# chanzuckerberg/shasta

Measured on NVIDIA H100. Metric: candidate_pairs_found_and_aligned_per_s, higher is better.
Workload: dtype u64/i32

## Files before the change

shasta_b200/csrc/align.cu:

```cuda
#include "context.cuh"
#include "align_kernels.cuh"
#include "hostpool.cuh"
#include "digest.cuh"

#include <algorithm>
#include <atomic>
#include <exception>
#include <memory>
#include <mutex>
#include <chrono>
#include <cstring>
#include <sys/mman.h>
#include <thread>
#include <limits>
#include <map>
#include <vector>

namespace shb {

extern thread_local uint64_t g_launchCount;

namespace {

uint32_t warpsForClass(const DpClass& k)
{
    if(k.c > 0) return kDpMaxWarpsPerBlock;
    const uint64_t perWarp = 3ull * (k.wMax + 1) * 4;
    const uint32_t w = uint32_t(std::min<uint64_t>(kDpMaxWarpsPerBlock, (200ull * 1024) / perWarp));
    return w ? w : 1;
}
size_t smemForClass(const DpClass& k, uint32_t warps) { return k.c > 0 ? 0 : size_t(warps) * 3 * (k.wMax + 1) * 4; }
size_t scanKernelSmemLimit()
{
    size_t most = 0;
    for(uint32_t k = 0; k < kDpClassCount; k++) most = std::max(most, smemForClass(dpClassAt(k), warpsForClass(dpClassAt(k))));
    return most;
}
constexpr uint32_t kMaxBandWidth = dpClassAt(kDpClassCount - 1).wMax;
struct DpLaunch { uint32_t blocks, threads; size_t smem; };
DpLaunch dpLaunch(const DpClass& k, uint32_t jobs)
{
    const uint32_t warps = warpsForClass(k);
    return DpLaunch{ceilDiv(jobs, warps * (32 / k.lanes)), warps * 32, smemForClass(k, warps)};
}

template<uint32_t K = 0, class... Args> void launchBanded(uint32_t k, const DpLaunch& l, cudaStream_t st, Args... args)
{
    if constexpr(K < kDpClassCount) {
        if(k != K) { launchBanded<K + 1>(k, l, st, args...); return; }
        constexpr DpClass cl = dpClassAt(K);
        if constexpr(cl.c == 0) {
            SHB_CUDA(cudaFuncSetAttribute(bandedAlignKernel<32, 0>, cudaFuncAttributeMaxDynamicSharedMemorySize, int(scanKernelSmemLimit())));
        }
        auto* kernel = &bandedAlignKernel<int(cl.lanes), int(cl.c)>;
        SHB_LAUNCH(kernel, l.blocks, l.threads, l.smem, st, args...);
    }
}
template<uint32_t K = 0, class... Args> void launchStage1Forward(uint32_t k, uint32_t jobs, cudaStream_t st, Args... args)
{
    if constexpr(K < kDpForwardClassCount) {
        if(k != K) { launchStage1Forward<K + 1>(k, jobs, st, args...); return; }
        constexpr DpForwardClass f = dpForwardClassAt(K);
        auto* kernel = &method3Stage1ForwardKernel<int(f.lanes), int(f.rows)>;
        SHB_LAUNCH(kernel, ceilDiv(jobs, kDpMaxWarpsPerBlock * (32 / f.lanes)), kDpMaxWarpsPerBlock * 32, 0, st, args...);
    }
}

struct Batch {
    DeviceBuffer<uint32_t> cand, counts, infoWords, jobKeep, jobBytes, keep, keepIndex, bytes32, selected;
    DeviceBuffer<DpJob> jobs1, jobs;
    DeviceBuffer<unsigned long long> tw, twOff, outCnt, outOff, bytes64, bytesOff, scanWs64;
    DeviceBuffer<uint32_t> trace;
    DeviceBuffer<uint2> ordinals, runs;
    DeviceBuffer<int2> endCells;
    DeviceBuffer<uint32_t> runCounts;
    DeviceBuffer<unsigned long long> cellCnt, cellOff;
    DeviceBuffer<uint32_t> gridCounts, gridAux, gridList, componentCount, jobOffsets;
    DeviceBuffer<uint8_t> gridFlags;
    DeviceBuffer<int32_t> gridBands;
    DeviceBuffer<uint32_t> orderValsA, orderValsB;
    DeviceBuffer<uint64_t> orderKeysA, orderKeysB;
    const uint32_t* order = nullptr;
};

enum WorkerScalar { kScTotal64 = 0, kScTotal32 = 1, kScSkipped = 2, kScForwardCells = 3, kScTooWide = 4, kScBandCells = 5,
                    kScDigits = 16, kScCount = 16 + 256 };

struct AlignWorker {
    cudaStream_t stream = nullptr;
    static constexpr int kSideStreams = 3;
    cudaStream_t side[kSideStreams] = {nullptr, nullptr, nullptr};
    cudaEvent_t forkEv = nullptr, joinEv[kSideStreams] = {nullptr, nullptr, nullptr};
    static constexpr int kHiStreams = 4;
    cudaStream_t hiStream[kHiStreams] = {nullptr, nullptr, nullptr, nullptr};
    cudaEvent_t hiJoinEv[kHiStreams] = {nullptr, nullptr, nullptr, nullptr};
    std::vector<cudaEvent_t> unitEvents;
    cudaEvent_t dp1a = nullptr, dp1b = nullptr, dp2a = nullptr, dp2b = nullptr;
    Batch batch;
    SortWorkspace sortWs;
    DeviceBuffer<uint32_t> scanWs;
    DeviceBuffer<unsigned long long> scalars;
    double dpMs = 0.;
    uint64_t traceWords = 0, launches = 0;

    void init()
    {
        if(stream) return;
        int least = 0, greatest = 0;
        SHB_CUDA(cudaDeviceGetStreamPriorityRange(&least, &greatest));
        SHB_CUDA(cudaStreamCreateWithFlags(&stream, cudaStreamNonBlocking));
        SHB_CUDA(cudaEventCreateWithFlags(&forkEv, cudaEventDisableTiming));
        for(int i = 0; i < kSideStreams; i++) {
            SHB_CUDA(cudaStreamCreateWithFlags(&side[i], cudaStreamNonBlocking));
            SHB_CUDA(cudaEventCreateWithFlags(&joinEv[i], cudaEventDisableTiming));
        }
        for(int i = 0; i < kHiStreams; i++) {
            SHB_CUDA(cudaStreamCreateWithPriority(&hiStream[i], cudaStreamNonBlocking, greatest));
            SHB_CUDA(cudaEventCreateWithFlags(&hiJoinEv[i], cudaEventDisableTiming));
        }
        SHB_CUDA(cudaEventCreate(&dp1a)); SHB_CUDA(cudaEventCreate(&dp1b));
        SHB_CUDA(cudaEventCreate(&dp2a)); SHB_CUDA(cudaEventCreate(&dp2b));
        scalars.reserve(kScCount);
    }
    ~AlignWorker()
    {
        for(int i = 0; i < kHiStreams; i++) { if(hiStream[i]) cudaStreamDestroy(hiStream[i]); if(hiJoinEv[i]) cudaEventDestroy(hiJoinEv[i]); }
        for(cudaEvent_t e : unitEvents) cudaEventDestroy(e);
        for(int i = 0; i < kSideStreams; i++) { if(side[i]) cudaStreamDestroy(side[i]); if(joinEv[i]) cudaEventDestroy(joinEv[i]); }
        for(cudaEvent_t e : {forkEv, dp1a, dp1b, dp2a, dp2b}) if(e) cudaEventDestroy(e);
        if(stream) cudaStreamDestroy(stream);
    }
    unsigned long long* sc(int k) { return scalars.get() + k; }
};

struct AlignCache {
    DeviceBuffer<uint64_t> dsToc;
    DeviceBuffer<uint32_t> dsKmer, dsOrdinal;
    uint32_t dsMaxRow = 0, dsK = 0;
    double dsFactor = -1.;
    uint64_t dsGeneration = ~0ull;
    DeviceBuffer<uint32_t> sortedKmer, sortedOrdinal;
    uint64_t sortedGeneration = ~0ull;
    uint64_t lengthCheckGeneration = ~0ull;
    uint64_t longestRead = 0;
    std::vector<std::unique_ptr<AlignWorker>> workers;
    DeviceBuffer<uint32_t> outRecords;
    DeviceBuffer<unsigned long long> outToc;
    DeviceBuffer<uint8_t> outData;
    cudaStream_t finalStream = nullptr;
    double lastBytesPerCandidate = 0.;
    ~AlignCache() { if(finalStream) cudaStreamDestroy(finalStream); }
};

AlignCache& cache(shb_context* c)
{
    if(!c->alignCache) c->alignCache = new AlignCache();
    return *static_cast<AlignCache*>(c->alignCache);
}

template<class F> void forEachClassConcurrently(AlignWorker& w, const std::vector<uint64_t>& classCounts, uint32_t chunkMax, F launch)
{
    cudaStream_t st = w.stream;
    struct Unit { int k; uint32_t count; uint64_t offset; };
    std::vector<Unit> units;
    const int classCount = int(classCounts.size());
    std::vector<uint64_t> offsets(classCounts.size(), 0);
    for(int k = 1; k < classCount; k++) offsets[k] = offsets[k-1] + classCounts[k-1];
    for(int k = classCount - 1; k >= 0; k--) {
        const uint64_t count = classCounts[k];
        if(!count) continue;
        const uint64_t chunks = (count + chunkMax - 1) / chunkMax, per = (count + chunks - 1) / chunks;
        for(uint64_t begin = 0; begin < count; begin += per) units.push_back({k, uint32_t(std::min(per, count - begin)), offsets[k] + begin});
    }
    if(units.empty()) return;
    constexpr int kStreams = AlignWorker::kSideStreams + 1;
    bool used[AlignWorker::kSideStreams] = {false, false, false};
    if(units.size() > 1) SHB_CUDA(cudaEventRecord(w.forkEv, st));
    for(size_t u = 0; u < units.size(); u++) {
        const int i = (u + 1 == units.size()) ? kStreams - 1 : int(u % kStreams);
        cudaStream_t s = st;
        if(i < AlignWorker::kSideStreams) {
            s = w.side[i];
            if(!used[i]) { SHB_CUDA(cudaStreamWaitEvent(s, w.forkEv, 0)); used[i] = true; }
        }
        launch(units[u].k, units[u].count, units[u].offset, s);
    }
    for(int i = 0; i < AlignWorker::kSideStreams; i++) {
        if(!used[i]) continue;
        SHB_CUDA(cudaEventRecord(w.joinEv[i], w.side[i]));
        SHB_CUDA(cudaStreamWaitEvent(st, w.joinEv[i], 0));
    }
}

void buildDownsampled(shb_context* c, uint32_t k, double factor)
{
    AlignCache& ds = cache(c);
    if(ds.dsK == k && ds.dsFactor == factor && ds.dsGeneration == c->markerGeneration && ds.dsToc.get()) return;
    cudaStream_t st = c->stream;
    const uint64_t M = c->localMarkerCount;
    const uint32_t rows = uint32_t(2 * c->readCountTotal);
    const uint32_t hashThreshold = uint32_t(factor * double(std::numeric_limits<uint32_t>::max()));
    ds.dsToc.reserve(uint64_t(rows) + 1);
    const uint32_t chunk = envCount("SHB_DOWNSAMPLE_CHUNK", 1u << 27);
    c->flagsBuf.reserve(std::min<uint64_t>(chunk, M) + 1);
    c->indexBuf.reserve(std::min<uint64_t>(chunk, M) + 1);
    c->scanWs.reserve(scanWorkspaceElements(chunk));
    uint32_t* totalDev = reinterpret_cast<uint32_t*>(c->scalar(kSlotDownsampleTotal));
// ... 645 lines not shown
```

shasta_b200/csrc/align_kernels.cuh:

```cuda
#pragma once

#include "common.cuh"
#include "../../include/shb_dp_policy.h"

namespace shb {

__device__ __forceinline__ uint32_t reverseComplementKmerId(uint32_t kmer, uint32_t k)
{
    const uint32_t mask = (k == 16) ? 0xffffu : ((1u << k) - 1u);
    const uint32_t lsb = ~kmer & mask;
    const uint32_t msb = ~(kmer >> k) & mask;
    return ((__brev(msb) >> (32 - k)) << k) | (__brev(lsb) >> (32 - k));
}

__device__ __forceinline__ uint32_t kmerDownsamplingHash(uint32_t kmer, uint32_t k)
{
    const uint64_t n = uint64_t(kmer) + uint64_t(reverseComplementKmerId(kmer, k));
    const uint32_t m = 0x5bd1e995u;
    uint32_t h = 13477u ^ 8u;
    uint32_t k1 = uint32_t(n);
    k1 *= m; k1 ^= k1 >> 24; k1 *= m;
    h *= m; h ^= k1;
    uint32_t k2 = uint32_t(n >> 32);
    k2 *= m; k2 ^= k2 >> 24; k2 *= m;
    h *= m; h ^= k2;
    h ^= h >> 13; h *= m; h ^= h >> 15;
    return h;
}

static __global__ void downsampleFlagsKernel(const uint32_t* __restrict__ kmerIds, uint64_t begin, uint32_t n,
                                             uint32_t k, uint32_t hashThreshold, uint32_t* __restrict__ flags)
{
    const uint32_t i = blockIdx.x * blockDim.x + threadIdx.x;
    if(i >= n) return;
    flags[i] = (kmerDownsamplingHash(kmerIds[begin + i], k) < hashThreshold) ? 1u : 0u;
}

static __global__ void downsampleCompactKernel(const uint32_t* __restrict__ kmerIds, uint64_t begin, uint32_t n,
                                               const uint32_t* __restrict__ flags, const uint32_t* __restrict__ index,
                                               const uint64_t* __restrict__ toc, uint32_t orientedReadCount, uint64_t dsBase,
                                               uint32_t* __restrict__ dsKmer, uint32_t* __restrict__ dsOrdinal)
{
    const uint32_t i = blockIdx.x * blockDim.x + threadIdx.x;
    if(i >= n || !flags[i]) return;
    const uint64_t p = begin + i;
    uint32_t lo = 0, hi = orientedReadCount;
    while(hi - lo > 1) {
        const uint32_t mid = lo + ((hi - lo) >> 1);
        if(toc[mid] <= p) lo = mid; else hi = mid;
    }
    const uint64_t d = dsBase + index[i];
    dsKmer[d] = kmerIds[p];
    dsOrdinal[d] = uint32_t(p - toc[lo]);
}

static __global__ void downsampleTocKernel(const uint64_t* __restrict__ toc, uint32_t orientedReadCount,
                                           uint64_t begin, uint32_t n, const uint32_t* __restrict__ index,
                                           uint64_t dsBase, uint64_t dsTotalAfterChunk, uint64_t* __restrict__ dsToc)
{
    const uint32_t o = blockIdx.x * blockDim.x + threadIdx.x;
    if(o > orientedReadCount) return;
    const uint64_t p = toc[o];
    if(p >= begin && p < begin + n) dsToc[o] = dsBase + index[p - begin];
    else if(p == begin + n) dsToc[o] = dsTotalAfterChunk;
}

struct DpJob {
    uint64_t aOffset, bOffset;
    uint32_t nx, ny;
    int32_t lo, hi;
    uint64_t traceOffset;
    uint64_t outOffset;
    uint32_t state;
    uint32_t pad;
};
constexpr uint32_t kStateRun = 0, kStateEmpty = 1, kStateSkipped = 2;

struct DpScores { int32_t match, mismatch, gap; };

constexpr uint32_t kCandidateStrand0Bit = 0x100u;
__device__ __forceinline__ void candidateOrientedReads(const uint32_t* __restrict__ candidates, uint64_t p, uint64_t& o0, uint64_t& o1)
{
    const uint32_t r0 = candidates[3ull * p], r1 = candidates[3ull * p + 1], w = candidates[3ull * p + 2];
    const uint32_t strand0 = (w & kCandidateStrand0Bit) ? 1u : 0u;
    const bool same = (w & 0xffu) != 0;
    o0 = 2ull * r0 + strand0;
    o1 = 2ull * r1 + (same ? strand0 : 1u - strand0);
}

constexpr int32_t kNegInf = -(1 << 29);
constexpr int kDpMaxWarpsPerBlock = 4;

__device__ __forceinline__ bool dpViaGap(int32_t g, int32_t diag) { return SHB_DP_DIAG_WINS_TIES ? (g > diag) : (g >= diag); }
__device__ __forceinline__ bool dpHorzWins(int32_t horzIn, int32_t vertIn) { return SHB_DP_VERT_BEFORE_HORZ ? (horzIn > vertIn) : (horzIn >= vertIn); }
__device__ __forceinline__ bool dpEndCellBetter(int32_t s2, int32_t i2, int32_t j2, int32_t s, int32_t i, int32_t j)
{
    if(s2 != s) return s2 > s;
    return SHB_DP_END_FIRST_MAX ? (i2 < i || (i2 == i && j2 < j)) : (i2 > i || (i2 == i && j2 > j));
}
constexpr int32_t kEndCellNone = SHB_DP_END_FIRST_MAX ? 0x7fffffff : -1;

struct DpClass { uint32_t wMax, lanes, c; };
constexpr uint32_t kDpClassCount = 17, kDpGroupClassCount = 7;
__host__ __device__ constexpr DpClass dpClassAt(uint32_t k)
{
    const uint32_t m = k - kDpGroupClassCount;
    const uint32_t warpC = m < 2 ? m + 3u : m < 4 ? 2u * m + 2u : 4u * m - 4u;
    return k < kDpGroupClassCount ? DpClass{16u * (k + 2u), 8u, k + 2u}
         : m < 6 ? DpClass{64u * warpC, 32u, warpC}
         : DpClass{2048u << (m - 6u), 32u, 0u};
}
struct DpShape { uint32_t cls, lanes, c, wpad; };
__host__ __device__ inline DpShape dpBandShape(int32_t lo, int32_t hi)
{
    const uint32_t need = uint32_t(hi - lo + 1) + 2u;
    uint32_t k = 0;
    while(k + 1 < kDpClassCount && need > dpClassAt(k).wMax) k++;
    const DpClass cl = dpClassAt(k);
    return DpShape{k, cl.lanes, cl.c, (need + 2u * cl.lanes - 1u) & ~(2u * cl.lanes - 1u)};
}
constexpr int32_t kGapBarrier = -(1 << 28);
__host__ __device__ inline int32_t dpFirstColumn(int32_t lo) { return lo > 0 ? lo : 0; }
__host__ __device__ inline int32_t dpLastColumn(uint32_t nx, uint32_t ny, int32_t hi)
{
    const int64_t bottom = int64_t(ny) + hi;
    return int32_t(bottom < int64_t(nx) ? bottom : int64_t(nx));
}
struct DpTraceSteps {
    int32_t iFirst;
    uint32_t reciprocal;
    __host__ __device__ uint32_t step(int32_t i, uint32_t p) const { return uint32_t(i - iFirst) + ((p * reciprocal) >> 16); }
};
__host__ __device__ inline DpTraceSteps dpTraceSteps(const DpShape& s, int32_t lo)
{
    return s.c ? DpTraceSteps{dpFirstColumn(lo), (65536u + 2u * s.c - 1u) / (2u * s.c)} : DpTraceSteps{0, 0u};
}
__host__ __device__ inline uint64_t dpTraceWords(uint32_t nx, uint32_t ny, int32_t lo, int32_t hi)
{
    const DpShape s = dpBandShape(lo, hi);
    uint64_t columns = nx;
    if(s.c) {
        const int64_t active = int64_t(dpLastColumn(nx, ny, hi)) - dpFirstColumn(lo);
        columns = uint64_t(active > 0 ? active : 0);
    }
    return ((columns + s.lanes + 15u) / 16u + 1u) * s.wpad;
}

__device__ inline void bandedOverlapDp(const uint32_t* __restrict__ a, uint32_t nx, const uint32_t* __restrict__ b, uint32_t ny,
                                       int32_t lo, int32_t hi, DpScores sc,
                                       int32_t* hPrev, int32_t* hCur, uint32_t* traceAcc, uint32_t* __restrict__ trace,
                                       int32_t& bestScore, int32_t& bestI, int32_t& bestJ)
{
    const unsigned lane = threadIdx.x & 31u;
    const int32_t W = hi - lo + 1;
    const int32_t Wpad = int32_t(dpBandShape(lo, hi).wpad);
    const int32_t chunks = Wpad >> 5;

    bestScore = kNegInf * 2; bestI = -1; bestJ = -1;
    for(int32_t e = lane; e <= Wpad; e += 32) { hPrev[e] = kNegInf; hCur[e] = kNegInf; }
    for(int32_t e = lane; e < Wpad; e += 32) traceAcc[e] = 0;
    __syncwarp();

    for(int32_t i = 0; i <= int32_t(nx); i++) {
        const uint32_t ai = (i > 0) ? a[i - 1] : 0u;
        int32_t carry = kNegInf;
        int32_t carryP = kNegInf * 2;
        const bool lastColumn = (i == int32_t(nx));
        const int32_t eLastRow = int32_t(ny) - i + hi;
        for(int32_t c = 0; c < chunks; c++) {
            const int32_t e = (c << 5) + int32_t(lane);
            const int32_t j = e + i - hi;
            const bool valid = (e < W) && (j >= 0) && (j <= int32_t(ny));
            int32_t A = kNegInf, diag = kNegInf, horz = kNegInf;
            const bool boundary = (i == 0) || (j == 0);
            if(valid) {
                if(boundary) A = 0;
                else {
                    diag = hPrev[e] + ((ai == b[j - 1]) ? sc.match : sc.mismatch);
                    horz = hPrev[e + 1] + sc.gap;
                    A = max(diag, horz);
                }
            }
            int32_t P = A - e * sc.gap;
#pragma unroll
            for(int d = 1; d < 32; d <<= 1) {
                const int32_t t = __shfl_up_sync(0xffffffffu, P, d);
                if(lane >= (unsigned)d) P = max(P, t);
            }
            P = max(P, carryP);
            int32_t H = P + e * sc.gap;
            if(!valid) H = kNegInf;
            if(valid && boundary) H = 0;
            int32_t below = __shfl_up_sync(0xffffffffu, H, 1);
            if(lane == 0) below = carry;
            uint32_t code = 0;
            if(valid && !boundary) {
                const int32_t vert = below + sc.gap;
                const bool horzWins = dpHorzWins(horz, vert);
                code = dpViaGap(max(horz, vert), diag) ? (horzWins ? 3u : 1u) : 0u;
            }
            hCur[e] = H;
            uint32_t acc = (traceAcc[e] << 2) | code;
            traceAcc[e] = acc;
            if((i & 15) == 15 || lastColumn) {
                const uint32_t filled = uint32_t(i & 15) + 1u;
                if(e + 1 < Wpad) trace[uint64_t(i >> 4) * uint32_t(Wpad) + uint32_t(e + 1)] = acc << (2u * (16u - filled));
                traceAcc[e] = 0;
            }
            carry = __shfl_sync(0xffffffffu, H, 31);
            carryP = __shfl_sync(0xffffffffu, P, 31);
            if(lastColumn) {
                int32_t mx = valid ? H : kNegInf * 2;
#pragma unroll
                for(int d = 16; d > 0; d >>= 1) mx = max(mx, __shfl_xor_sync(0xffffffffu, mx, d));
                const unsigned who = __ballot_sync(0xffffffffu, valid && H == mx);
                if(who && (SHB_DP_END_FIRST_MAX ? (mx > bestScore) : (mx >= bestScore))) {
                    const int pick = SHB_DP_END_FIRST_MAX ? (__ffs(who) - 1) : (31 - __clz(who));
                    bestScore = mx; bestI = i; bestJ = ((c << 5) + pick) + i - hi;
                }
            } else if(eLastRow >= (c << 5) && eLastRow < (c << 5) + 32 && eLastRow < W && eLastRow >= 0) {
                const int32_t s = __shfl_sync(0xffffffffu, H, eLastRow & 31);
                if(SHB_DP_END_FIRST_MAX ? (s > bestScore) : (s >= bestScore)) { bestScore = s; bestI = i; bestJ = int32_t(ny); }
            }
        }
        __syncwarp();
        int32_t* t = hPrev; hPrev = hCur; hCur = t;
    }
}

template<int C> struct SubChunkLimits { int32_t first[C]; int32_t gap[C]; };

template<int C> __device__ __forceinline__ void initSubChunkLimits(SubChunkLimits<C>& lim, int32_t p0, int32_t W, int32_t hi, int32_t gap)
{
#pragma unroll
    for(int c = 0; c < C; c++) {
        const int32_t e = p0 + c - 1;
        lim.first[c] = (e >= 0 && e < W) ? max(0, hi - e) : 0x7fffffff;
        lim.gap[c] = (e == -1 || e == W) ? kGapBarrier : gap;
    }
}


struct FmaUnits { int32_t one, two, four; };
constexpr int kDpInPlaceTraceMaxC = 4;
__device__ __forceinline__ int32_t fmaPipeAdd(int32_t a, int32_t b, int32_t one)
{
    int32_t r;
    asm("mad.lo.s32 %0, %1, %2, %3;" : "=r"(r) : "r"(a), "r"(one), "r"(b));
    return r;
}
__device__ __forceinline__ uint32_t fmaPipeMul(uint32_t a, uint32_t b)
{
    uint32_t r;
    asm("mad.lo.u32 %0, %1, %2, 0;" : "=r"(r) : "r"(a), "r"(b));
    return r;
}
__device__ __forceinline__ void fmaPipeAddIfEqual(int32_t& acc, uint32_t x, uint32_t y, int32_t v, int32_t one)
{
    asm("{\n\t.reg .pred q;\n\tsetp.eq.u32 q, %1, %2;\n\t@q mad.lo.s32 %0, %3, %4, %0;\n\t}" : "+r"(acc) : "r"(x), "r"(y), "r"(v), "r"(one));
}
template<bool OrEqual> __device__ __forceinline__ void fmaPipeAddIfGreater(uint32_t& acc, int32_t x, int32_t y, int32_t a, int32_t b)
{
    if(OrEqual) asm("{\n\t.reg .pred q;\n\tsetp.ge.s32 q, %1, %2;\n\t@q mad.lo.u32 %0, %3, %4, %0;\n\t}" : "+r"(acc) : "r"(x), "r"(y), "r"(a), "r"(b));
    else asm("{\n\t.reg .pred q;\n\tsetp.gt.s32 q, %1, %2;\n\t@q mad.lo.u32 %0, %3, %4, %0;\n\t}" : "+r"(acc) : "r"(x), "r"(y), "r"(a), "r"(b));
}

template<int C, bool Boundary, int Step = -1> __device__ __forceinline__ void systolicSubChunk(
    int32_t (&H)[C], uint32_t (&Tr)[C], const SubChunkLimits<C>& lim, int32_t i, uint32_t ai,
    int32_t below , int32_t top , const uint32_t* bw, DpScores sc, FmaUnits u)
{
    constexpr int32_t kCodeUnit = (Step >= 0) ? int32_t(1u << (2 * (15 - (Step >= 0 ? Step : 0)))) : 1;
    int32_t vertIn = below;
    const int32_t matchBonus = sc.match - sc.mismatch;
#pragma unroll
    for(int c = 0; c < C; c++) {
        int32_t diag = fmaPipeAdd(H[c], sc.mismatch, u.one);
        fmaPipeAddIfEqual(diag, ai, bw[c], matchBonus, u.one);
        const int32_t horzIn = (c + 1 < C) ? H[c + 1] : top;
        const int32_t gapIn = max(vertIn, horzIn);
        int32_t h = __viaddmax_s32(gapIn, lim.gap[c], diag);
        uint32_t tr = (Step >= 0) ? Tr[c] : fmaPipeMul(Tr[c], uint32_t(u.four));
        if(Step >= 0) {
            if(SHB_DP_DIAG_WINS_TIES) fmaPipeAddIfGreater<false>(tr, h, diag, u.one, kCodeUnit);
            else fmaPipeAddIfGreater<true>(tr, fmaPipeAdd(gapIn, lim.gap[c], u.one), diag, u.one, kCodeUnit);
            fmaPipeAddIfGreater<!SHB_DP_VERT_BEFORE_HORZ>(tr, horzIn, vertIn, u.one, 2 * kCodeUnit);
        } else {
            if(SHB_DP_DIAG_WINS_TIES) fmaPipeAddIfGreater<false>(tr, h, diag, u.one, u.one);
            else fmaPipeAddIfGreater<true>(tr, fmaPipeAdd(gapIn, lim.gap[c], u.one), diag, u.one, u.one);
            fmaPipeAddIfGreater<!SHB_DP_VERT_BEFORE_HORZ>(tr, horzIn, vertIn, u.one, u.two);
        }
        Tr[c] = tr;
        if(Boundary) h = (i == lim.first[c]) ? 0 : h;
        H[c] = h;
        vertIn = h;
    }
}

template<int C> __device__ __forceinline__ void systolicEndCells(
    const int32_t (&H)[C], const SubChunkLimits<C>& lim, int32_t e0, int32_t i, int32_t cStar ,
    int32_t nx, int32_t& bestScore, int32_t& bestI, int32_t& bestJ)
{
#pragma unroll
    for(int c = 0; c < C; c++) {
        const bool lastRow = (c == cStar);
        const bool lastColumn = (i == nx) && (c <= cStar) && (lim.first[c] <= nx);
        if((lastRow || lastColumn) && i >= lim.first[c]) {
            const int32_t h = H[c];
            const int32_t jPlusHi = e0 + c + i;
            if(dpEndCellBetter(h, i, jPlusHi, bestScore, bestI, bestJ)) { bestScore = h; bestI = i; bestJ = jPlusHi; }
        }
    }
}

template<int C> struct SystolicState {
    int32_t HA[C], HB[C];
    uint32_t TA[C], TB[C];
    SubChunkLimits<C> limA, limB;
    uint32_t bw[2 * C];
    int32_t i;
    const uint32_t* ap;
    const uint32_t* bNext;
    int32_t jNext;
    int32_t bestScore, bestI, bestJ;
};

template<int G, int C, bool Checked, int Step> __device__ __forceinline__ void systolicStep(
    SystolicState<C>& s, int32_t eA, int32_t eB, int32_t rowEndA, int32_t nx, int32_t ny, DpScores sc, FmaUnits fu)
{
    uint32_t ai = 0xfffffffeu;
    uint32_t bIn = 0xffffffffu;
    if(Checked) {
        if(uint32_t(s.i - 1) < uint32_t(nx)) ai = __ldg(s.ap);
        if(uint32_t(s.jNext) < uint32_t(ny)) bIn = __ldg(s.bNext);
    } else {
        ai = __ldg(s.ap);
        bIn = __ldg(s.bNext);
    }
    const int32_t below = __shfl_up_sync(0xffffffffu, s.HB[C - 1], 1, G);
    systolicSubChunk<C, Checked, Step>(s.HA, s.TA, s.limA, s.i, ai, below, s.HB[0], s.bw, sc, fu);
    const int32_t top = __shfl_down_sync(0xffffffffu, s.HA[0], 1, G);
    systolicSubChunk<C, Checked, Step>(s.HB, s.TB, s.limB, s.i, ai, s.HA[C - 1], top, s.bw + C, sc, fu);
    if(Checked) {
        const int32_t cStar = rowEndA - s.i;
        if((uint32_t(cStar) < uint32_t(2 * C) || s.i == nx) && uint32_t(s.i) <= uint32_t(nx)) {
            systolicEndCells<C>(s.HA, s.limA, eA, s.i, cStar, nx, s.bestScore, s.bestI, s.bestJ);
            systolicEndCells<C>(s.HB, s.limB, eB, s.i, cStar - C, nx, s.bestScore, s.bestI, s.bestJ);
        }
    }
#pragma unroll
    for(int k = 0; k + 1 < 2 * C; k++) s.bw[k] = s.bw[k + 1];
    s.bw[2 * C - 1] = bIn;
    s.i++; s.ap++; s.bNext++; s.jNext++;
}

template<int G, int C, bool Checked, int... Steps> __device__ __forceinline__ void systolicStepsInPlace(
    SystolicState<C>& s, int32_t eA, int32_t eB, int32_t rowEndA, int32_t nx, int32_t ny, DpScores sc, FmaUnits fu,
    std::integer_sequence<int, Steps...>)
{
    (systolicStep<G, C, Checked, Steps>(s, eA, eB, rowEndA, nx, ny, sc, fu), ...);
}

template<int G, int C, bool Checked> __device__ __forceinline__ void systolicBlock(
    SystolicState<C>& s, int32_t eA, int32_t eB, int32_t rowEndA, int32_t nx, int32_t ny, DpScores sc, FmaUnits fu)
{
    if constexpr(C <= kDpInPlaceTraceMaxC) {
#pragma unroll
        for(int c = 0; c < C; c++) { s.TA[c] = 0; s.TB[c] = 0; }
        systolicStepsInPlace<G, C, Checked>(s, eA, eB, rowEndA, nx, ny, sc, fu, std::make_integer_sequence<int, 16>{});
    } else {
        constexpr int kUnroll = (C <= 4) ? 4 : (C <= 8) ? 2 : 1;
#pragma unroll kUnroll
        for(int step = 0; step < 16; step++) systolicStep<G, C, Checked, -1>(s, eA, eB, rowEndA, nx, ny, sc, fu);
    }
}

template<int G, int C> __device__ inline void bandedOverlapDpSystolic(
    const uint32_t* __restrict__ a, uint32_t nxU, const uint32_t* __restrict__ b, uint32_t nyU, int32_t lo, int32_t hi, bool live,
    DpScores sc, FmaUnits fu, uint32_t* __restrict__ trace, int32_t& bestScore, int32_t& bestI, int32_t& bestJ)
{
    const int32_t lane = int32_t(threadIdx.x & unsigned(G - 1));
    const int32_t nx = int32_t(nxU), ny = int32_t(nyU);
    const int32_t W = hi - lo + 1;
    const uint32_t WpadJob = dpBandShape(lo, hi).wpad;
    SystolicState<C> s;
    const int32_t pA = (2 * lane) * C, pB = (2 * lane + 1) * C;
    const int32_t eA = pA - 1, eB = pB - 1;
#pragma unroll
    for(int c = 0; c < C; c++) { s.HA[c] = kNegInf; s.HB[c] = kNegInf; s.TA[c] = 0; s.TB[c] = 0; }
    initSubChunkLimits<C>(s.limA, pA, W, hi, sc.gap);
    initSubChunkLimits<C>(s.limB, pB, W, hi, sc.gap);
    s.bestScore = kNegInf * 2; s.bestI = kEndCellNone; s.bestJ = kEndCellNone;
    const int32_t iFirst = dpFirstColumn(lo), iLast = dpLastColumn(nxU, nyU, hi);
    s.i = iFirst - lane;
    const int32_t jA = eA + s.i - hi;
    s.ap = a + (int64_t(s.i) - 1);
#pragma unroll
    for(int k = 0; k < 2 * C; k++) {
        const int32_t idx = jA - 1 + k;
        s.bw[k] = 0xffffffffu;
        if(uint32_t(idx) < uint32_t(ny)) s.bw[k] = __ldg(b + idx);
    }
    s.jNext = jA - 1 + 2 * C;
    s.bNext = b + int64_t(s.jNext);
    const int32_t rowEndA = ny + hi - eA;
    const int32_t blocks = live ? (iLast - iFirst + G + 15) >> 4 : 0;
    int32_t headBlocks = live ? ((max(0, hi) - iFirst + G - 1) >> 4) + 1 : INT32_MAX;
    const int32_t firstEndStep = min(nx - iFirst, ny + hi - iFirst - 2 * G * C + G);
    int32_t tailBlock = max(0, firstEndStep) >> 4;
    int32_t warpBlocks = blocks;
    if constexpr(G < 32) {
        headBlocks = __reduce_max_sync(0xffffffffu, headBlocks);
        tailBlock = __reduce_min_sync(0xffffffffu, tailBlock);
        warpBlocks = __reduce_max_sync(0xffffffffu, blocks);
    }
    uint32_t* row = trace;
    for(int32_t blk = 0; blk < warpBlocks; blk++, row += WpadJob) {
        if(blk < headBlocks || blk >= tailBlock) systolicBlock<G, C, true>(s, eA, eB, rowEndA, nx, ny, sc, fu);
        else systolicBlock<G, C, false>(s, eA, eB, rowEndA, nx, ny, sc, fu);
        if(blk < blocks) {
#pragma unroll
            for(int c = 0; c < C; c++) {
                if(uint32_t(pA + c) < WpadJob) row[pA + c] = s.TA[c];
                if(uint32_t(pB + c) < WpadJob) row[pB + c] = s.TB[c];
            }
        }
    }
    bestScore = s.bestScore; bestI = s.bestI; bestJ = s.bestJ;
    if(bestI != kEndCellNone) bestJ -= hi;
#pragma unroll
    for(int d = G / 2; d > 0; d >>= 1) {
        const int32_t s2 = __shfl_xor_sync(0xffffffffu, bestScore, d);
        const int32_t i2 = __shfl_xor_sync(0xffffffffu, bestI, d);
        const int32_t j2 = __shfl_xor_sync(0xffffffffu, bestJ, d);
        if(dpEndCellBetter(s2, i2, j2, bestScore, bestI, bestJ)) { bestScore = s2; bestI = i2; bestJ = j2; }
    }
    if(bestI == kEndCellNone) { bestI = -1; bestJ = -1; }
    __syncwarp();
}

struct Method3Args {
    const uint32_t* candidates;
    uint64_t candidateBegin; uint32_t n;
    const uint32_t* order;
    const uint64_t* toc;
    const uint64_t* dsToc; const uint32_t* dsKmer; const uint32_t* dsOrdinal;
    DpScores scores;
    int32_t bandExtend, maxBand;
};

__device__ inline void setStage2Band(DpJob& j2, bool diagonalStep, int32_t offsetMin, int32_t offsetMax, int32_t bandExtend, int32_t maxBand)
{
    if(!diagonalStep) { j2.state = kStateEmpty; return; }
    const int32_t bandMin = int32_t(uint32_t(offsetMin) - uint32_t(bandExtend));
    const int32_t bandMax = int32_t(uint32_t(offsetMax) + uint32_t(bandExtend));
    if(int32_t(uint32_t(bandMax) - uint32_t(bandMin)) > maxBand) j2.state = kStateEmpty;
    else if(bandMin > bandMax || bandMax < -int32_t(j2.ny) || bandMin > int32_t(j2.nx)) j2.state = kStateSkipped;
    else {
        j2.lo = max(bandMin, -int32_t(j2.ny));
        j2.hi = min(bandMax, int32_t(j2.nx));
        j2.state = kStateRun;
    }
}

template<int G> __device__ __forceinline__ bool dpGroupJob(const uint32_t* __restrict__ order, uint32_t n, const DpJob* __restrict__ jobs,
                                                           uint32_t& warpSlot, uint32_t& p, DpJob& job, bool& live)
{
    warpSlot = (blockIdx.x * (blockDim.x >> 5) + (threadIdx.x >> 5)) * (32u / G);
    if(warpSlot >= n) return false;
    const uint32_t slot = warpSlot + (threadIdx.x & 31u) / G;
    live = false;
    p = 0;
    if(slot < n) {
        p = order[slot];
        job = jobs[p];
        live = job.state == kStateRun;
    }
    if(!live) { job = DpJob{}; job.state = kStateEmpty; }
    return __any_sync(0xffffffffu, live);
}

constexpr int dpMinBlocks(int C) { return C <= 2 ? 6 : C == 3 ? 5 : C == 4 ? 4 : C <= 8 ? 2 : 1; }

constexpr uint32_t kPairNoDiagonalStep = 0x7fff7fffu;
constexpr uint32_t kPairNoMatchingStep = 0x7fff7ffeu;
constexpr uint32_t kStage1ForwardMaxRows = 512;
constexpr uint32_t kStage1ForwardMaxMarkers = 32000;

__device__ __forceinline__ uint32_t packedAdd16(uint32_t x, uint32_t y)
{
    uint32_t r;
    asm("add.s16x2 %0, %1, %2;" : "=r"(r) : "r"(x), "r"(y));
    return r;
}
__device__ __forceinline__ uint32_t packOffsetPair(int32_t lowHalf, int32_t highHalf)
{
    return (uint32_t(lowHalf) & 0xffffu) | (uint32_t(highHalf) << 16);
}

template<int G, int R> __global__ void __launch_bounds__(kDpMaxWarpsPerBlock * 32)
method3Stage1ForwardKernel(Method3Args g, const DpJob* __restrict__ jobs1, DpJob* __restrict__ jobs2)
{
    const int32_t lane = int32_t(threadIdx.x & unsigned(G - 1));
    uint32_t warpSlot, p;
    DpJob job;
    bool live;
    if(!dpGroupJob<G>(g.order, g.n, jobs1, warpSlot, p, job, live)) return;
    const uint32_t* __restrict__ a = g.dsKmer + job.aOffset;
    const uint32_t* __restrict__ oa = g.dsOrdinal + job.aOffset;
    const int32_t nx = int32_t(job.nx), ny = int32_t(job.ny);
    const DpScores sc = g.scores;

    uint32_t bk[R], boP[R];
    int32_t H[R];
    uint32_t P[R];
#pragma unroll
    for(int r = 0; r < R; r++) {
        const int32_t j = R * lane + r + 1;
        bk[r] = 0xffffffffu; boP[r] = 0;
        if(j <= ny) {
            bk[r] = __ldg(g.dsKmer + job.bOffset + (j - 1));
            const int32_t ob = int32_t(__ldg(g.dsOrdinal + job.bOffset + (j - 1)));
            boP[r] = packOffsetPair(-ob, ob);
        }
        H[r] = 0; P[r] = kPairNoDiagonalStep;
    }
    const int32_t lastLane = live ? (ny - 1) / R : 0, rLast = live ? (ny - 1) % R : -1;
    int32_t upH = 0;
    uint32_t upP = kPairNoDiagonalStep;
    int32_t bestScore = 0, bestI = kEndCellNone, bestJ = kEndCellNone;
    uint32_t bestP = kPairNoDiagonalStep;

    int32_t steps = nx + lastLane;
    if constexpr(G < 32) steps = __reduce_max_sync(0xffffffffu, steps);
#pragma unroll 2
    for(int32_t t = 0; t < steps; t++) {
        int32_t inH = __shfl_up_sync(0xffffffffu, H[R - 1], 1, G);
        uint32_t inP = __shfl_up_sync(0xffffffffu, P[R - 1], 1, G);
        if(lane == 0) { inH = 0; inP = kPairNoDiagonalStep; }
        const int32_t i = t - lane + 1;
        if(uint32_t(i - 1) < uint32_t(nx)) {
            const uint32_t ai = __ldg(a + (i - 1));
            const int32_t ao = int32_t(__ldg(oa + (i - 1)));
            const uint32_t aoP = packOffsetPair(ao, -ao);
            int32_t dH = upH; uint32_t dP = upP;
            int32_t vH = inH; uint32_t vP = inP;
#pragma unroll
            for(int r = 0; r < R; r++) {
                const int32_t hH = H[r]; const uint32_t hP = P[r];
                const bool eq = (ai == bk[r]);
                const int32_t diag = dH + (eq ? sc.match : sc.mismatch);
                const int32_t gapIn = max(vH, hH);
                const int32_t h = __viaddmax_s32(gapIn, sc.gap, diag);
                const bool viaGap = SHB_DP_DIAG_WINS_TIES ? (h > diag) : (gapIn + sc.gap >= diag), viaHorz = dpHorzWins(hH, vH);
                const uint32_t stepP = __vmins2(dP, eq ? packedAdd16(aoP, boP[r]) : kPairNoMatchingStep);
                const uint32_t gapP = viaHorz ? hP : vP;
                const uint32_t pr = viaGap ? gapP : stepP;
                dH = hH; dP = hP;
                vH = h; vP = pr;
                H[r] = h; P[r] = pr;
            }
            if(lane == lastLane && i != nx) {
                int32_t h = 0; uint32_t pr = 0;
                switch(rLast) {
#define SHB_PICK_ROW(k) case k: if constexpr(k < R) { h = H[k]; pr = P[k]; } break;
                SHB_PICK_ROW(0) SHB_PICK_ROW(1) SHB_PICK_ROW(2) SHB_PICK_ROW(3) SHB_PICK_ROW(4) SHB_PICK_ROW(5) SHB_PICK_ROW(6) SHB_PICK_ROW(7)
                SHB_PICK_ROW(8) SHB_PICK_ROW(9) SHB_PICK_ROW(10) SHB_PICK_ROW(11) SHB_PICK_ROW(12) SHB_PICK_ROW(13) SHB_PICK_ROW(14) SHB_PICK_ROW(15)
#undef SHB_PICK_ROW
                default: break;
                }
                if(SHB_DP_END_FIRST_MAX ? (h > bestScore) : (h >= bestScore)) { bestScore = h; bestI = i; bestJ = ny; bestP = pr; }
            }
            if(i == nx) {
#pragma unroll
                for(int r = 0; r < R; r++) {
                    const int32_t j = R * lane + r + 1;
                    if(j <= ny && (SHB_DP_END_FIRST_MAX ? (H[r] > bestScore) : (H[r] >= bestScore))) { bestScore = H[r]; bestI = i; bestJ = j; bestP = P[r]; }
                }
            }
        }
        upH = inH; upP = inP;
    }
    if constexpr(!SHB_DP_END_FIRST_MAX) {
        if(lane == 0 && dpEndCellBetter(0, nx, 0, bestScore, bestI, bestJ)) { bestScore = 0; bestI = nx; bestJ = 0; bestP = kPairNoDiagonalStep; }
    }
#pragma unroll
    for(int d = G / 2; d > 0; d >>= 1) {
        const int32_t s2 = __shfl_xor_sync(0xffffffffu, bestScore, d);
        const int32_t i2 = __shfl_xor_sync(0xffffffffu, bestI, d);
        const int32_t j2 = __shfl_xor_sync(0xffffffffu, bestJ, d);
        const uint32_t p2 = __shfl_xor_sync(0xffffffffu, bestP, d);
        if(dpEndCellBetter(s2, i2, j2, bestScore, bestI, bestJ)) {
            bestScore = s2; bestI = i2; bestJ = j2; bestP = p2;
        }
    }
    if(lane == 0 && live) {
        DpJob j2 = jobs2[p];
        const uint32_t lowHalf = bestP & 0xffffu;
        const bool noMatch = lowHalf == (kPairNoMatchingStep & 0xffffu);
        setStage2Band(j2, bestI != kEndCellNone && lowHalf != (kPairNoDiagonalStep & 0xffffu),
                      noMatch ? INT32_MAX : int32_t(int16_t(lowHalf)), noMatch ? INT32_MIN : -int32_t(int16_t(bestP >> 16)),
                      g.bandExtend, g.maxBand);
        jobs2[p] = j2;
    }
}

struct BandedArgs {
    uint32_t n;
    const uint32_t* order;
    const uint32_t* kmerIds;
    DpScores scores;
    FmaUnits fma;
    uint32_t wMax;
};

template<int G, int C> __global__ void __launch_bounds__(kDpMaxWarpsPerBlock * 32, dpMinBlocks(C))
bandedAlignKernel(BandedArgs g, const DpJob* __restrict__ jobs, uint32_t* __restrict__ trace, int2* __restrict__ endCells)
{
    extern __shared__ int32_t smem[];
    const unsigned warp = threadIdx.x >> 5, lane = threadIdx.x & unsigned(G - 1);
    uint32_t warpSlot, p;
    DpJob job;
    bool live;
    if(!dpGroupJob<G>(g.order, g.n, jobs, warpSlot, p, job, live)) return;
    const uint32_t* a = g.kmerIds + job.aOffset;
    const uint32_t* b = g.kmerIds + job.bOffset;
    int32_t bestScore, bestI, bestJ;
    if constexpr(C > 0) {
        bandedOverlapDpSystolic<G, C>(a, job.nx, b, job.ny, job.lo, job.hi, live, g.scores, g.fma, live ? trace + job.traceOffset : nullptr,
                                      bestScore, bestI, bestJ);
        (void)warp;
    } else {
        static_assert(C > 0 || G == 32, "the scan kernel runs one job per warp");
        const uint32_t stride = g.wMax + 1;
        int32_t* hPrev = smem + warp * 3 * stride;
        int32_t* hCur = hPrev + stride;
        uint32_t* traceAcc = reinterpret_cast<uint32_t*>(hCur + stride);
        bandedOverlapDp(a, job.nx, b, job.ny, job.lo, job.hi, g.scores, hPrev, hCur, traceAcc, trace + job.traceOffset,
                        bestScore, bestI, bestJ);
    }
    if(lane == 0 && live) endCells[p] = make_int2(bestI, bestJ);
}

constexpr uint32_t kRunLengthShift = 28, kRunOrdinalMask = (1u << kRunLengthShift) - 1u;

__device__ __forceinline__ void prefetchL1(const void* p) { asm volatile("prefetch.global.L1 [%0];" :: "l"(p)); }

static __global__ void __launch_bounds__(128)
tracebackKernel(uint32_t n, const uint32_t* __restrict__ order, const DpJob* __restrict__ jobs, const int2* __restrict__ endCells,
                const uint32_t* __restrict__ trace, uint2* __restrict__ runs, uint32_t* __restrict__ runCounts)
{
    const uint32_t slot = blockIdx.x * blockDim.x + threadIdx.x;
    if(slot >= n) return;
    const uint32_t p = order[slot];
    const DpJob job = jobs[p];
    const int2 end = endCells[p];
    int32_t i = end.x, j = end.y;
    uint32_t count = 0;
    if(job.state == kStateRun && i > 0 && j > 0) {
        const DpShape shape = dpBandShape(job.lo, job.hi);
        const uint32_t Wpad = shape.wpad;
        const DpTraceSteps steps = dpTraceSteps(shape, job.lo);
        const uint32_t* __restrict__ tr = trace + job.traceOffset;
        uint2* __restrict__ out = runs + job.outOffset;
        const int32_t hi = job.hi;
        uint32_t lastBlock = 0xffffffffu;
        while(i > 0 && j > 0) {
            const uint32_t off = uint32_t(j - i + hi) + 1u;
            const uint32_t t = steps.step(i, off);
            const uint32_t block = t >> 4;
            const uint32_t word = tr[uint64_t(block) * Wpad + off];
            if(block != lastBlock) {
                lastBlock = block;
                if(block >= 1) prefetchL1(tr + uint64_t(block - 1) * Wpad + off);
                if(block >= 2) prefetchL1(tr + uint64_t(block - 2) * Wpad + off);
            }
            const uint32_t q = t & 15u;
            const uint32_t w = word >> (2u * (15u - q));
            const uint32_t gaps = w & 0x55555555u & (q == 15u ? 0xffffffffu : ((1u << (2u * (q + 1u))) - 1u));
            const int32_t run = min(gaps ? ((__ffs(int(gaps)) - 1) >> 1) : int32_t(q) + 1, min(i, j));
            if(run > 0) {
                out[count++] = make_uint2(uint32_t(i - 1) | (uint32_t(run - 1) << kRunLengthShift), uint32_t(j - 1));
                i -= run; j -= run;
            } else if(w & 2u) i--;
            else j--;
        }
    }
    runCounts[p] = count;
}

static __global__ void __launch_bounds__(128)
filterStepsKernel(uint32_t n, const uint32_t* __restrict__ order, const DpJob* __restrict__ jobs, const uint32_t* __restrict__ kmerIds,
                  const uint2* __restrict__ runs, const uint32_t* __restrict__ runCounts, uint2* __restrict__ ordinals,
                  uint32_t* __restrict__ counts)
{
    const uint32_t slot = blockIdx.x * (blockDim.x >> 5) + (threadIdx.x >> 5);
    if(slot >= n) return;
    const uint32_t lane = threadIdx.x & 31u;
    const uint32_t p = order[slot];
    const DpJob job = jobs[p];
    const uint32_t* __restrict__ a = kmerIds + job.aOffset;
    const uint32_t* __restrict__ b = kmerIds + job.bOffset;
    const uint2* __restrict__ in = runs + job.outOffset;
    uint2* __restrict__ out = ordinals + job.outOffset;
    const uint32_t nRuns = runCounts[p];
    uint32_t count = 0;
    for(uint32_t base = 0; base < nRuns; base += 32) {
        const uint32_t r = base + lane;
        uint2 d = make_uint2(0, 0);
        uint32_t length = 0;
        if(r < nRuns) { d = in[r]; length = (d.x >> kRunLengthShift) + 1u; }
        const uint32_t x0 = d.x & kRunOrdinalMask, y0 = d.y;
        uint32_t inclusive = length;
#pragma unroll
        for(int s = 1; s < 32; s <<= 1) {
            const uint32_t v = __shfl_up_sync(0xffffffffu, inclusive, s);
            if(lane >= uint32_t(s)) inclusive += v;
        }
        const uint32_t total = __shfl_sync(0xffffffffu, inclusive, 31);
        const uint32_t first = inclusive - length;
        for(uint32_t s0 = 0; s0 < total; s0 += 32) {
            const uint32_t step = s0 + lane;
            uint32_t owner = 0;
#pragma unroll
            for(int w = 16; w > 0; w >>= 1) {
                const uint32_t probe = owner + uint32_t(w);
                const uint32_t v = __shfl_sync(0xffffffffu, first, int(probe & 31u));
                if(v <= step) owner = probe;
            }
            const uint32_t k = step - __shfl_sync(0xffffffffu, first, int(owner));
            const uint32_t x = __shfl_sync(0xffffffffu, x0, int(owner)) - k;
            const uint32_t y = __shfl_sync(0xffffffffu, y0, int(owner)) - k;
            const bool keep = step < total && a[x] == b[y];
            const unsigned m = __ballot_sync(0xffffffffu, keep);
            if(keep) out[count + __popc(m & ((1u << lane) - 1u))] = make_uint2(x, y);
            count += __popc(m);
        }
    }
    if(lane == 0) counts[p] = count;
}

static __global__ void __launch_bounds__(128)
stage1BandKernel(uint32_t n, const uint32_t* __restrict__ order, const DpJob* __restrict__ jobs1, const uint32_t* __restrict__ dsOrdinal,
                 const uint2* __restrict__ ordinals, const uint32_t* __restrict__ runCounts, const uint32_t* __restrict__ counts,
                 int32_t bandExtend, int32_t maxBand, DpJob* __restrict__ jobs2)
{
    const uint32_t slot = blockIdx.x * (blockDim.x >> 5) + (threadIdx.x >> 5);
    if(slot >= n) return;
    const uint32_t lane = threadIdx.x & 31u;
    const uint32_t p = order[slot];
    const DpJob j1 = jobs1[p];
    const uint32_t* __restrict__ oa = dsOrdinal + j1.aOffset;
    const uint32_t* __restrict__ ob = dsOrdinal + j1.bOffset;
    const uint2* __restrict__ kept = ordinals + j1.outOffset;
    const uint32_t count = counts[p];
    int32_t offsetMin = INT32_MAX, offsetMax = INT32_MIN;
    for(uint32_t k = lane; k < count; k += 32) {
        const uint2 s = kept[k];
        const int32_t off = int32_t(oa[s.x]) - int32_t(ob[s.y]);
        offsetMin = min(offsetMin, off);
        offsetMax = max(offsetMax, off);
    }
#pragma unroll
    for(int d = 16; d > 0; d >>= 1) {
        offsetMin = min(offsetMin, __shfl_xor_sync(0xffffffffu, offsetMin, d));
        offsetMax = max(offsetMax, __shfl_xor_sync(0xffffffffu, offsetMax, d));
    }
    if(lane == 0) {
        DpJob j2 = jobs2[p];
        setStage2Band(j2, runCounts[p] != 0, offsetMin, offsetMax, bandExtend, maxBand);
        jobs2[p] = j2;
    }
}

struct FilterOptions {
    uint64_t minAlignedMarkerCount, maxSkip, maxDrift, maxTrim;
    double minAlignedFraction;
    uint32_t suppressContainments;
};

__device__ __forceinline__ uint32_t compressedStreakBytes(int32_t skip0, int32_t skip1, uint32_t len)
{
// ... 784 lines not shown
```

Before: 11.44 million.

## Allow uneven per-lane band spans to add finer group band classes

After: 11.80 million, median of 6. +3.1%, better.

```diff
diff --git a/shasta_b200/csrc/align.cu b/shasta_b200/csrc/align.cu
--- a/shasta_b200/csrc/align.cu
+++ b/shasta_b200/csrc/align.cu
@@ -50,9 +50,9 @@
         if(k != K) { launchBanded<K + 1>(k, l, st, args...); return; }
         constexpr DpClass cl = dpClassAt(K);
         if constexpr(cl.c == 0) {
-            SHB_CUDA(cudaFuncSetAttribute(bandedAlignKernel<32, 0>, cudaFuncAttributeMaxDynamicSharedMemorySize, int(scanKernelSmemLimit())));
-        }
-        auto* kernel = &bandedAlignKernel<int(cl.lanes), int(cl.c)>;
+            SHB_CUDA(cudaFuncSetAttribute(bandedAlignKernel<32, 0, 0>, cudaFuncAttributeMaxDynamicSharedMemorySize, int(scanKernelSmemLimit())));
+        }
+        auto* kernel = &bandedAlignKernel<int(cl.lanes), int(cl.c), int(cl.span - cl.c)>;
         SHB_LAUNCH(kernel, l.blocks, l.threads, l.smem, st, args...);
     }
 }
diff --git a/shasta_b200/csrc/align_kernels.cuh b/shasta_b200/csrc/align_kernels.cuh
--- a/shasta_b200/csrc/align_kernels.cuh
+++ b/shasta_b200/csrc/align_kernels.cuh
@@ -100,24 +100,26 @@
 }
 constexpr int32_t kEndCellNone = SHB_DP_END_FIRST_MAX ? 0x7fffffff : -1;
 
-struct DpClass { uint32_t wMax, lanes, c; };
-constexpr uint32_t kDpClassCount = 17, kDpGroupClassCount = 7;
+struct DpClass { uint32_t wMax, lanes, c, span; };
+constexpr uint32_t kDpClassCount = 19, kDpGroupClassCount = 9;
 __host__ __device__ constexpr DpClass dpClassAt(uint32_t k)
 {
     const uint32_t m = k - kDpGroupClassCount;
     const uint32_t warpC = m < 2 ? m + 3u : m < 4 ? 2u * m + 2u : 4u * m - 4u;
-    return k < kDpGroupClassCount ? DpClass{16u * (k + 2u), 8u, k + 2u}
-         : m < 6 ? DpClass{64u * warpC, 32u, warpC}
-         : DpClass{2048u << (m - 6u), 32u, 0u};
-}
-struct DpShape { uint32_t cls, lanes, c, wpad; };
+    const uint32_t span = k < 4 ? k + 4u : 2u * k;
+    return k < kDpGroupClassCount ? DpClass{8u * span, 8u, span / 2u, span}
+         : m < 6 ? DpClass{64u * warpC, 32u, warpC, 2u * warpC}
+         : DpClass{2048u << (m - 6u), 32u, 0u, 0u};
+}
+struct DpShape { uint32_t cls, lanes, c, span, wpad; };
 __host__ __device__ inline DpShape dpBandShape(int32_t lo, int32_t hi)
 {
     const uint32_t need = uint32_t(hi - lo + 1) + 2u;
     uint32_t k = 0;
     while(k + 1 < kDpClassCount && need > dpClassAt(k).wMax) k++;
     const DpClass cl = dpClassAt(k);
-    return DpShape{k, cl.lanes, cl.c, (need + 2u * cl.lanes - 1u) & ~(2u * cl.lanes - 1u)};
+    const uint32_t unit = cl.lanes < 32 ? cl.lanes : 2u * cl.lanes;
+    return DpShape{k, cl.lanes, cl.c, cl.span, (need + unit - 1u) & ~(unit - 1u)};
 }
 constexpr int32_t kGapBarrier = -(1 << 28);
 __host__ __device__ inline int32_t dpFirstColumn(int32_t lo) { return lo > 0 ? lo : 0; }
@@ -133,7 +135,7 @@
 };
 __host__ __device__ inline DpTraceSteps dpTraceSteps(const DpShape& s, int32_t lo)
 {
-    return s.c ? DpTraceSteps{dpFirstColumn(lo), (65536u + 2u * s.c - 1u) / (2u * s.c)} : DpTraceSteps{0, 0u};
+    return s.c ? DpTraceSteps{dpFirstColumn(lo), (65536u + s.span - 1u) / s.span} : DpTraceSteps{0, 0u};
 }
 __host__ __device__ inline uint64_t dpTraceWords(uint32_t nx, uint32_t ny, int32_t lo, int32_t hi)
 {
@@ -312,11 +314,13 @@
     }
 }
 
-template<int C> struct SystolicState {
-    int32_t HA[C], HB[C];
-    uint32_t TA[C], TB[C];
-    SubChunkLimits<C> limA, limB;
-    uint32_t bw[2 * C];
+template<int C, int CB> struct SystolicState {
+    static constexpr int S = C + CB;
+    int32_t HA[C], HB[CB];
+    uint32_t TA[C], TB[CB];
+    SubChunkLimits<C> limA;
+    SubChunkLimits<CB> limB;
+    uint32_t bw[S];
     int32_t i;
     const uint32_t* ap;
     const uint32_t* bNext;
@@ -324,8 +328,8 @@
     int32_t bestScore, bestI, bestJ;
 };
 
-template<int G, int C, bool Checked, int Step> __device__ __forceinline__ void systolicStep(
-    SystolicState<C>& s, int32_t eA, int32_t eB, int32_t rowEndA, int32_t nx, int32_t ny, DpScores sc, FmaUnits fu)
+template<int G, int C, int CB, bool Checked, int Step> __device__ __forceinline__ void systolicStep(
+    SystolicState<C, CB>& s, int32_t eA, int32_t eB, int32_t rowEndA, int32_t nx, int32_t ny, DpScores sc, FmaUnits fu)
 {
     uint32_t ai = 0xfffffffeu;
     uint32_t bIn = 0xffffffffu;
@@ -336,45 +340,47 @@
         ai = __ldg(s.ap);
         bIn = __ldg(s.bNext);
     }
-    const int32_t below = __shfl_up_sync(0xffffffffu, s.HB[C - 1], 1, G);
+    const int32_t below = __shfl_up_sync(0xffffffffu, s.HB[CB - 1], 1, G);
     systolicSubChunk<C, Checked, Step>(s.HA, s.TA, s.limA, s.i, ai, below, s.HB[0], s.bw, sc, fu);
     const int32_t top = __shfl_down_sync(0xffffffffu, s.HA[0], 1, G);
-    systolicSubChunk<C, Checked, Step>(s.HB, s.TB, s.limB, s.i, ai, s.HA[C - 1], top, s.bw + C, sc, fu);
+    systolicSubChunk<CB, Checked, Step>(s.HB, s.TB, s.limB, s.i, ai, s.HA[C - 1], top, s.bw + C, sc, fu);
     if(Checked) {
         const int32_t cStar = rowEndA - s.i;
-        if((uint32_t(cStar) < uint32_t(2 * C) || s.i == nx) && uint32_t(s.i) <= uint32_t(nx)) {
+        if((uint32_t(cStar) < uint32_t(C + CB) || s.i == nx) && uint32_t(s.i) <= uint32_t(nx)) {
             systolicEndCells<C>(s.HA, s.limA, eA, s.i, cStar, nx, s.bestScore, s.bestI, s.bestJ);
-            systolicEndCells<C>(s.HB, s.limB, eB, s.i, cStar - C, nx, s.bestScore, s.bestI, s.bestJ);
-        }
-    }
-#pragma unroll
-    for(int k = 0; k + 1 < 2 * C; k++) s.bw[k] = s.bw[k + 1];
-    s.bw[2 * C - 1] = bIn;
+            systolicEndCells<CB>(s.HB, s.limB, eB, s.i, cStar - C, nx, s.bestScore, s.bestI, s.bestJ);
+        }
+    }
+#pragma unroll
+    for(int k = 0; k + 1 < C + CB; k++) s.bw[k] = s.bw[k + 1];
+    s.bw[C + CB - 1] = bIn;
     s.i++; s.ap++; s.bNext++; s.jNext++;
 }
 
-template<int G, int C, bool Checked, int... Steps> __device__ __forceinline__ void systolicStepsInPlace(
-    SystolicState<C>& s, int32_t eA, int32_t eB, int32_t rowEndA, int32_t nx, int32_t ny, DpScores sc, FmaUnits fu,
+template<int G, int C, int CB, bool Checked, int... Steps> __device__ __forceinline__ void systolicStepsInPlace(
+    SystolicState<C, CB>& s, int32_t eA, int32_t eB, int32_t rowEndA, int32_t nx, int32_t ny, DpScores sc, FmaUnits fu,
     std::integer_sequence<int, Steps...>)
 {
-    (systolicStep<G, C, Checked, Steps>(s, eA, eB, rowEndA, nx, ny, sc, fu), ...);
-}
-
-template<int G, int C, bool Checked> __device__ __forceinline__ void systolicBlock(
-    SystolicState<C>& s, int32_t eA, int32_t eB, int32_t rowEndA, int32_t nx, int32_t ny, DpScores sc, FmaUnits fu)
+    (systolicStep<G, C, CB, Checked, Steps>(s, eA, eB, rowEndA, nx, ny, sc, fu), ...);
+}
+
+template<int G, int C, int CB, bool Checked> __device__ __forceinline__ void systolicBlock(
+    SystolicState<C, CB>& s, int32_t eA, int32_t eB, int32_t rowEndA, int32_t nx, int32_t ny, DpScores sc, FmaUnits fu)
 {
     if constexpr(C <= kDpInPlaceTraceMaxC) {
 #pragma unroll
-        for(int c = 0; c < C; c++) { s.TA[c] = 0; s.TB[c] = 0; }
-        systolicStepsInPlace<G, C, Checked>(s, eA, eB, rowEndA, nx, ny, sc, fu, std::make_integer_sequence<int, 16>{});
+        for(int c = 0; c < C; c++) s.TA[c] = 0;
+#pragma unroll
+        for(int c = 0; c < CB; c++) s.TB[c] = 0;
+        systolicStepsInPlace<G, C, CB, Checked>(s, eA, eB, rowEndA, nx, ny, sc, fu, std::make_integer_sequence<int, 16>{});
     } else {
         constexpr int kUnroll = (C <= 4) ? 4 : (C <= 8) ? 2 : 1;
 #pragma unroll kUnroll
-        for(int step = 0; step < 16; step++) systolicStep<G, C, Checked, -1>(s, eA, eB, rowEndA, nx, ny, sc, fu);
-    }
-}
-
-template<int G, int C> __device__ inline void bandedOverlapDpSystolic(
+        for(int step = 0; step < 16; step++) systolicStep<G, C, CB, Checked, -1>(s, eA, eB, rowEndA, nx, ny, sc, fu);
+    }
+}
+
+template<int G, int C, int CB> __device__ inline void bandedOverlapDpSystolic(
     const uint32_t* __restrict__ a, uint32_t nxU, const uint32_t* __restrict__ b, uint32_t nyU, int32_t lo, int32_t hi, bool live,
     DpScores sc, FmaUnits fu, uint32_t* __restrict__ trace, int32_t& bestScore, int32_t& bestI, int32_t& bestJ)
 {
@@ -382,30 +388,33 @@
     const int32_t nx = int32_t(nxU), ny = int32_t(nyU);
     const int32_t W = hi - lo + 1;
     const uint32_t WpadJob = dpBandShape(lo, hi).wpad;
-    SystolicState<C> s;
-    const int32_t pA = (2 * lane) * C, pB = (2 * lane + 1) * C;
+    constexpr int S = C + CB;
+    SystolicState<C, CB> s;
+    const int32_t pA = lane * S, pB = pA + C;
     const int32_t eA = pA - 1, eB = pB - 1;
 #pragma unroll
-    for(int c = 0; c < C; c++) { s.HA[c] = kNegInf; s.HB[c] = kNegInf; s.TA[c] = 0; s.TB[c] = 0; }
+    for(int c = 0; c < C; c++) { s.HA[c] = kNegInf; s.TA[c] = 0; }
+#pragma unroll
+    for(int c = 0; c < CB; c++) { s.HB[c] = kNegInf; s.TB[c] = 0; }
     initSubChunkLimits<C>(s.limA, pA, W, hi, sc.gap);
-    initSubChunkLimits<C>(s.limB, pB, W, hi, sc.gap);
+    initSubChunkLimits<CB>(s.limB, pB, W, hi, sc.gap);
     s.bestScore = kNegInf * 2; s.bestI = kEndCellNone; s.bestJ = kEndCellNone;
     const int32_t iFirst = dpFirstColumn(lo), iLast = dpLastColumn(nxU, nyU, hi);
     s.i = iFirst - lane;
     const int32_t jA = eA + s.i - hi;
     s.ap = a + (int64_t(s.i) - 1);
 #pragma unroll
-    for(int k = 0; k < 2 * C; k++) {
+    for(int k = 0; k < S; k++) {
         const int32_t idx = jA - 1 + k;
         s.bw[k] = 0xffffffffu;
         if(uint32_t(idx) < uint32_t(ny)) s.bw[k] = __ldg(b + idx);
     }
-    s.jNext = jA - 1 + 2 * C;
+    s.jNext = jA - 1 + S;
     s.bNext = b + int64_t(s.jNext);
     const int32_t rowEndA = ny + hi - eA;
     const int32_t blocks = live ? (iLast - iFirst + G + 15) >> 4 : 0;
     int32_t headBlocks = live ? ((max(0, hi) - iFirst + G - 1) >> 4) + 1 : INT32_MAX;
-    const int32_t firstEndStep = min(nx - iFirst, ny + hi - iFirst - 2 * G * C + G);
+    const int32_t firstEndStep = min(nx - iFirst, ny + hi - iFirst - G * S + G);
     int32_t tailBlock = max(0, firstEndStep) >> 4;
     int32_t warpBlocks = blocks;
     if constexpr(G < 32) {
@@ -415,12 +424,12 @@
     }
     uint32_t* row = trace;
     for(int32_t blk = 0; blk < warpBlocks; blk++, row += WpadJob) {
-        if(blk < headBlocks || blk >= tailBlock) systolicBlock<G, C, true>(s, eA, eB, rowEndA, nx, ny, sc, fu);
-        else systolicBlock<G, C, false>(s, eA, eB, rowEndA, nx, ny, sc, fu);
+        if(blk < headBlocks || blk >= tailBlock) systolicBlock<G, C, CB, true>(s, eA, eB, rowEndA, nx, ny, sc, fu);
+        else systolicBlock<G, C, CB, false>(s, eA, eB, rowEndA, nx, ny, sc, fu);
         if(blk < blocks) {
 #pragma unroll
-            for(int c = 0; c < C; c++) {
-                if(uint32_t(pA + c) < WpadJob) row[pA + c] = s.TA[c];
+            for(int c = 0; c < CB; c++) {
+                if(c < C && uint32_t(pA + c) < WpadJob) row[pA + c] = s.TA[c];
                 if(uint32_t(pB + c) < WpadJob) row[pB + c] = s.TB[c];
             }
         }
@@ -479,7 +488,7 @@
     return __any_sync(0xffffffffu, live);
 }
 
-constexpr int dpMinBlocks(int C) { return C <= 2 ? 6 : C == 3 ? 5 : C == 4 ? 4 : C <= 8 ? 2 : 1; }
+constexpr int dpMinBlocks(int span) { return span <= 4 ? 6 : span <= 6 ? 5 : span <= 9 ? 4 : span <= 16 ? 2 : 1; }
 
 constexpr uint32_t kPairNoDiagonalStep = 0x7fff7fffu;
 constexpr uint32_t kPairNoMatchingStep = 0x7fff7ffeu;
@@ -613,7 +622,7 @@
     uint32_t wMax;
 };
 
-template<int G, int C> __global__ void __launch_bounds__(kDpMaxWarpsPerBlock * 32, dpMinBlocks(C))
+template<int G, int C, int CB> __global__ void __launch_bounds__(kDpMaxWarpsPerBlock * 32, dpMinBlocks(C + CB))
 bandedAlignKernel(BandedArgs g, const DpJob* __restrict__ jobs, uint32_t* __restrict__ trace, int2* __restrict__ endCells)
 {
     extern __shared__ int32_t smem[];
@@ -626,7 +635,7 @@
     const uint32_t* b = g.kmerIds + job.bOffset;
     int32_t bestScore, bestI, bestJ;
     if constexpr(C > 0) {
-        bandedOverlapDpSystolic<G, C>(a, job.nx, b, job.ny, job.lo, job.hi, live, g.scores, g.fma, live ? trace + job.traceOffset : nullptr,
+        bandedOverlapDpSystolic<G, C, CB>(a, job.nx, b, job.ny, job.lo, job.hi, live, g.scores, g.fma, live ? trace + job.traceOffset : nullptr,
                                       bestScore, bestI, bestJ);
         (void)warp;
     } else {
```
